# FEDDLib/FEDDLib

Hardware: AMD Instinct MI355X
Metric: DoF/s assemble+solve, 3D P1-Laplace cube (higher is better)
Workload: dtype f64

## Files before the change

feddlib_amd/csrc/gmres.hip:

```cpp
#include "fedd_internal.hpp"
#include <rccl/rccl.h>
#include <algorithm>
#include <cmath>
#include <cstdlib>

namespace fedd {
namespace {

constexpr int MD_ROWS = 2048;
constexpr int MD_CG = 8;
constexpr int MD2_CG = 8;
constexpr int AX_ROWS = 512;

__device__ __forceinline__ double2 ld2c(const double* __restrict__ p, int64_t r, int64_t n) {
    if (r + 1 < n) return *reinterpret_cast<const double2*>(p + r);
    double2 v;
    v.x = r < n ? p[r] : 0.0;
    v.y = 0.0;
    return v;
}

__device__ __forceinline__ double2 ld2(const double* __restrict__ p, int64_t r, int64_t n) {
    if (r + 1 < n) {
        typedef double v2d __attribute__((ext_vector_type(2)));
// ... 718 lines not shown
    double* V = f.V;
    double* u = f.w0;
    double* wt = f.w1;
    double* r = f.r;
    const dim3 gn = f.gn, blk = f.blk;
    hipStream_t st = f.st;

    FEDD_TRY(f.start(wt, -1));
    if (!(f.beta0 > 0)) {
        f.report(its_out, relres_out);
        return 0;
    }
    LaggedCheck lag(f, 2);
    FEDD_TRY(lag.create());
    const int nblkd = (int)((n + 2047) / 2048);
    const int md2_gy = c->md2_gy > 0 ? c->md2_gy : (int)std::max<int64_t>(1, (2048 + nblkd - 1) / nblkd);
    bool converged = false;
    while (!converged && f.its < max_it) {
        hipLaunchKernelGGL(k_cycle_init, dim3(1), dim3(1), 0, st, S, o, m, (const double*)(S + o.nrm + 3));
        hipLaunchKernelGGL(k_scale_to, gn, blk, 0, st, (const double*)r, (const double*)(S + o.misc + 1), V, n);
        FEDD_TRY(f.apply(V, u));
        {
            ScopedTimer t(c, FEDD_T_ORTHO);
            hipLaunchKernelGGL(k_multidot, dim3(nblk, 1), blk, 0, st, (const double*)V, ldv, n, 1, (const double*)u,
                               c->d_part.p, nblk, (const int32_t*)nullptr);
            hipLaunchKernelGGL(k_reduce_cols, dim3(1), blk, 0, st, (const double*)c->d_part.p, S + o2.hp, nblk,
                               (const int32_t*)nullptr);
            FEDD_TRY(allreduce_sum(c, S + o2.hp, 1));
            hipLaunchKernelGGL(k_multiaxpy, dim3(nblk2), blk, 0, st, (const double*)V, ldv, n, 1, (const double*)(S + o2.hp),
                               u, c->d_part.p, (const int32_t*)nullptr);
            t.stop();
        }
        lag.begin_cycle();
        int stop = 0;
        for (int j = 0; j < m && lag.issued < max_it && !stop; ++j) {
            const int k = j + 1;
            FEDD_TRY(f.apply(u, wt, true));
            {
                ScopedTimer t(c, FEDD_T_ORTHO);
                const int ncg = (k + 1 + MD2_CG - 1) / MD2_CG;
                ScopedTimer td(c, FEDD_T_GS_DOT);
                td.bytes(8.0 * (double)n * (k + 2));
                hipLaunchKernelGGL(k_multidot2<4>, dim3(nblkd, std::min(md2_gy, ncg)), blk, 0, st, (const double*)V, ldv, n,
                                   k, (const double*)u, (const double*)wt, c->d_part.p, nblkd);
                td.stop();
                hipLaunchKernelGGL(k_reduce_cols, dim3(2 * k + 2), blk, 0, st, (const double*)c->d_part.p, S + o2.st, nblkd,
                                   (const int32_t*)nullptr);
                FEDD_TRY(allreduce_sum(c, S + o2.st, 2 * k + 2));
                hipLaunchKernelGGL(k_dcgs2_small, dim3(1), blk, (size_t)(6 * m + 8) * sizeof(double), st, S, o, o2, k, m,
                                   c->h_pinned_dev ? c->h_pinned_dev + 4 * (j & 1) : (double*)nullptr);
                if (k < m) {
                    ScopedTimer tu(c, FEDD_T_GS_UPDATE);
                    tu.bytes(8.0 * (double)n * (k + 4));
                    hipLaunchKernelGGL(k_axpy2, dim3(nblk2), blk, 0, st, V, ldv, n, k, (const double*)(S + o2.cf), m, u,
                                       (const double*)wt);
                    tu.stop();
                }
                t.stop();
            }
            FEDD_TRY(lag.record(j, !c->h_pinned_dev, &stop));
        }
        FEDD_TRY(lag.drain(&stop));
        converged = stop == 1;
        const bool broke = stop == 2;
        FEDD_TRY(f.add_correction(lag.cols, call.x));
        if (!converged && (f.its < max_it || broke)) {
            FEDD_TRY(f.true_residual(call.x, r, false, -1, f.project));
            if (broke) {
                double ta = 0.0;
                FEDD_TRY(f.read_norm(&ta));
                f.relres = ta / f.beta0;
                if (f.relres <= call.rtol) converged = true;
            }
        }
    }
    return f.finish(its_out, relres_out);
}


constexpr int ss_cg(int S) { return S >= 16 ? 2 : 4; }

template <int OFF>
__device__ __forceinline__ double xchg_add(double lo, double hi, int lane) {
    if constexpr (OFF == 32 || OFF == 16) {
        const unsigned l0 = __double2loint(lo), l1 = __double2hiint(lo), h0 = __double2loint(hi), h1 = __double2hiint(hi);
        if constexpr (OFF == 32) {
            const auto r0 = __builtin_amdgcn_permlane32_swap(l0, h0, false, false);
            const auto r1 = __builtin_amdgcn_permlane32_swap(l1, h1, false, false);
            return __hiloint2double(r1[0], r0[0]) + __hiloint2double(r1[1], r0[1]);
        } else {
            const auto r0 = __builtin_amdgcn_permlane16_swap(l0, h0, false, false);
            const auto r1 = __builtin_amdgcn_permlane16_swap(l1, h1, false, false);
            return __hiloint2double(r1[0], r0[0]) + __hiloint2double(r1[1], r0[1]);
        }
    } else {
        const bool up = (lane & OFF) != 0;
        const double keep = up ? hi : lo;
        const double send = up ? lo : hi;
        return keep + __shfl_xor(send, OFF, 64);
    }
}

template <int NV, int OFF, int W>
__device__ __forceinline__ void wave_reduce_step(double (&a)[NV], int lane) {
    if constexpr (W > 1) {
#pragma unroll
        for (int i = 0; i < W / 2; ++i) a[i] = xchg_add<OFF>(a[i], a[i + W / 2], lane);
    } else {
        a[0] += __shfl_xor(a[0], OFF, 64);
    }
    if constexpr (OFF > 1) wave_reduce_step<NV, OFF / 2, (W > 1 ? W / 2 : 1)>(a, lane);
}
template <int NV>
__device__ __forceinline__ double wave_reduce_transpose(double (&a)[NV], int lane) {
    wave_reduce_step<NV, 32, NV>(a, lane);
    return a[0];
}

struct RowPair {
    int64_t rc;
    bool v0, v1;
};
__device__ __forceinline__ RowPair row_pair(int64_t r, int64_t n) {
    RowPair q;
    q.v0 = r < n;
    q.v1 = r + 1 < n;
    q.rc = q.v0 ? r : 0;
    return q;
}
template <bool NT>
__device__ __forceinline__ double2 ldraw(const double* __restrict__ p, const RowPair& q) {
    typedef double v2d __attribute__((ext_vector_type(2)));
    const v2d t = NT ? __builtin_nontemporal_load(reinterpret_cast<const v2d*>(p + q.rc)) : *reinterpret_cast<const v2d*>(p + q.rc);
    return double2{t.x, t.y};
}
template <bool NT>
__device__ __forceinline__ double2 ldp(const double* __restrict__ p, const RowPair& q) {
    typedef double v2d __attribute__((ext_vector_type(2)));
    const v2d t = NT ? __builtin_nontemporal_load(reinterpret_cast<const v2d*>(p + q.rc)) : *reinterpret_cast<const v2d*>(p + q.rc);
    double2 v;
    v.x = q.v0 ? t.x : 0.0;
    v.y = q.v1 ? t.y : 0.0;
    return v;
}

constexpr int SS_LDS_GROUPS = 32;

template <int S, int NCH, int SS_CG>
__global__ __launch_bounds__(256) void k_blockdot(const double* __restrict__ V, int64_t ldv, int64_t n, int k, int sa_req,
                                                  const int32_t* __restrict__ d_sa, double* __restrict__ partial, int nblk) {
    constexpr int NV = SS_CG * S;
    static_assert(NV == 16 || NV == 32 || NV == 64, "block size");
    __shared__ double sh[SS_LDS_GROUPS][4][NV];
    const int sa = d_sa ? min(*d_sa, sa_req) : sa_req;
    if (sa <= 0) return;
    const int tid = threadIdx.x, lane = tid & 63, wave = tid >> 6;
    const int half = tid / 256, th = tid % 256;
    RowPair rp[NCH];
#pragma unroll
    for (int ch = 0; ch < NCH; ++ch)
        rp[ch] = row_pair((int64_t)blockIdx.x * (512 * NCH) + 512 * ch + 2 * th, n);
    double2 w[S][NCH];
#pragma unroll
    for (int j = 0; j < S; ++j)
#pragma unroll
        for (int ch = 0; ch < NCH; ++ch) {
            const int jj = half * S + j;
            const double2 t = ldp<false>(V + (int64_t)(k + (jj < sa ? jj : 0)) * ldv, rp[ch]);
            w[j][ch].x = jj < sa ? t.x : 0.0;
            w[j][ch].y = jj < sa ? t.y : 0.0;
        }
    const int ncol = k + sa;
    const int ncg = (ncol + SS_CG - 1) / SS_CG;
    int parked = 0, first_cg = blockIdx.y;
    constexpr int GRP = 64 / NV;
    auto flush = [&](int count) {
        __syncthreads();
        for (int e = tid; e < count * NV; e += 256) {
            const int g = e / NV, idx = e % NV;
            const int col = (first_cg + g * (int)gridDim.y) * SS_CG + idx / S;
            if (col < ncol) partial[((int64_t)col * S + (idx % S)) * nblk + blockIdx.x] = ((sh[g][0][idx] + sh[g][1][idx]) + sh[g][2][idx]) + sh[g][3][idx];
        }
        __syncthreads();
    };
    double2 v[SS_CG][NCH];
    auto load_group = [&](int cg) {
#pragma unroll
        for (int cc = 0; cc < SS_CG; ++cc) {
            const int col = cg * SS_CG + cc;
            const double* __restrict__ a = V + (int64_t)(col < ncol ? col : 0) * ldv;
#pragma unroll
            for (int ch = 0; ch < NCH; ++ch) {
                v[cc][ch] = col < k ? ldraw<true>(a, rp[ch]) : ldraw<false>(a, rp[ch]);
            }
        }
    };
    if ((int)blockIdx.y < ncg) load_group(blockIdx.y);
    for (int cg = blockIdx.y; cg < ncg; cg += gridDim.y) {
        double acc[NV];
#pragma unroll
        for (int cc = 0; cc < SS_CG; ++cc)
#pragma unroll
            for (int j = 0; j < S; ++j) {
                double s = 0.0;
#pragma unroll
                for (int ch = 0; ch < NCH; ++ch) s += v[cc][ch].x * w[j][ch].x + v[cc][ch].y * w[j][ch].y;
                acc[cc * S + j] = s;
            }
        if (cg + (int)gridDim.y < ncg) load_group(cg + gridDim.y);
        const double tot = wave_reduce_transpose<NV>(acc, lane);
        if ((lane & (GRP - 1)) == 0) sh[parked][wave][lane / GRP] = tot;
        if (++parked == SS_LDS_GROUPS) {
            flush(parked);
            parked = 0;
            first_cg = cg + gridDim.y;
        }
    }
    if (parked) flush(parked);
}

template <int S, bool COMB = false>
__global__ __launch_bounds__(256) void k_blockaxpy(double* __restrict__ V, int64_t ldv, int64_t n, int k, int sa_req,
                                                   const int32_t* __restrict__ d_sa, const double* __restrict__ cf,
                                                   const double* __restrict__ rinv, const double* __restrict__ yv = nullptr,
                                                   double* __restrict__ comb = nullptr) {
    const int sa = min(*d_sa, sa_req);
    if (sa <= 0) return;
    const int tid = threadIdx.x;
    const int64_t r = (int64_t)blockIdx.x * AX_ROWS + 2 * tid;
    const RowPair rp = row_pair(r, n);
    double2 cb = double2{0.0, 0.0};
    double2 acc[S];
#pragma unroll
    for (int j = 0; j < S; ++j) acc[j] = double2{0.0, 0.0};
    int c = 0;
    for (; c + 8 <= k; c += 8) {
        double2 q[8];
#pragma unroll
        for (int u = 0; u < 8; ++u) q[u] = ldp<true>(V + (int64_t)(c + u) * ldv, rp);
#pragma unroll
        for (int u = 0; u < 8; ++u) {
#pragma unroll
            for (int j = 0; j < S; ++j) {
                const double cc = cf[(c + u) * S + j];
                acc[j].x += cc * q[u].x;
                acc[j].y += cc * q[u].y;
            }
            if constexpr (COMB) {
                const double yc = yv[c + u];
                cb.x += yc * q[u].x;
                cb.y += yc * q[u].y;
            }
        }
    }
    for (; c < k; ++c) {
        const double2 q = ldp<true>(V + (int64_t)c * ldv, rp);
#pragma unroll
        for (int j = 0; j < S; ++j) {
            const double cc = cf[c * S + j];
            acc[j].x += cc * q.x;
            acc[j].y += cc * q.y;
        }
        if constexpr (COMB) {
            const double yc = yv[c];
            cb.x += yc * q.x;
            cb.y += yc * q.y;
        }
    }
    double2 t[S];
#pragma unroll
    for (int j = 0; j < S; ++j) {
        const double2 wv = ldp<false>(V + (int64_t)(k + (j < sa ? j : 0)) * ldv, rp);
        t[j].x = j < sa ? wv.x - acc[j].x : 0.0;
        t[j].y = j < sa ? wv.y - acc[j].y : 0.0;
    }
#pragma unroll
    for (int j = 0; j < S; ++j) {
        if (j < sa) {
            double2 o = double2{0.0, 0.0};
#pragma unroll
            for (int i = 0; i <= j; ++i) {
                const double ri = rinv[i * S + j];
                o.x += ri * t[i].x;
                o.y += ri * t[i].y;
            }
            double* wj = V + (int64_t)(k + j) * ldv;
            if (rp.v1) *reinterpret_cast<double2*>(wj + r) = o;
            else if (rp.v0) wj[r] = o.x;
            if constexpr (COMB) {
                if (j < sa - 1) {
                    const double yc = yv[k + j];
                    cb.x += yc * o.x;
                    cb.y += yc * o.y;
                }
            }
        }
    }
    if constexpr (COMB) {
        if (rp.v1) *reinterpret_cast<double2*>(comb + r) = cb;
        else if (rp.v0) comb[r] = cb.x;
    }
}

template <int S>
__global__ __launch_bounds__(256) void k_blockfuse(double* __restrict__ V, int64_t ldv, int64_t n, int k, int sa_req,
                                                   const int32_t* __restrict__ d_sa, const double* __restrict__ cf,
                                                   const double* __restrict__ rinv, double* __restrict__ partial, int nblk) {
    constexpr int SS_CG = 2, NV = SS_CG * S;
    static_assert(NV == 32, "block size");
    __shared__ double sh[SS_LDS_GROUPS][4][NV];
    const int sa = min(*d_sa, sa_req);
    if (sa <= 0) return;
    const int tid = threadIdx.x, lane = tid & 63, wave = tid >> 6;
    const int64_t r = (int64_t)blockIdx.x * AX_ROWS + 2 * tid;
    const RowPair rp = row_pair(r, n);
    double2 w[S];
    {
        double2 acc[S];
#pragma unroll
        for (int j = 0; j < S; ++j) acc[j] = double2{0.0, 0.0};
        int c = 0;
        for (; c + 8 <= k; c += 8) {
            double2 q[8];
#pragma unroll
            for (int u = 0; u < 8; ++u) q[u] = ldp<false>(V + (int64_t)(c + u) * ldv, rp);
#pragma unroll
            for (int u = 0; u < 8; ++u)
#pragma unroll
                for (int j = 0; j < S; ++j) {
                    const double cc = cf[(c + u) * S + j];
                    acc[j].x += cc * q[u].x;
                    acc[j].y += cc * q[u].y;
                }
        }
        for (; c < k; ++c) {
            const double2 q = ldp<false>(V + (int64_t)c * ldv, rp);
#pragma unroll
            for (int j = 0; j < S; ++j) {
                const double cc = cf[c * S + j];
                acc[j].x += cc * q.x;
                acc[j].y += cc * q.y;
            }
        }
#pragma unroll
        for (int j = 0; j < S; ++j) {
            const double2 wv = ldp<false>(V + (int64_t)(k + (j < sa ? j : 0)) * ldv, rp);
            acc[j].x = j < sa ? wv.x - acc[j].x : 0.0;
            acc[j].y = j < sa ? wv.y - acc[j].y : 0.0;
        }
#pragma unroll
        for (int j = 0; j < S; ++j) {
            double2 o = double2{0.0, 0.0};
            if (j < sa) {
#pragma unroll
                for (int i = 0; i <= j; ++i) {
                    const double ri = rinv[i * S + j];
                    o.x += ri * acc[i].x;
                    o.y += ri * acc[i].y;
                }
                double* wj = V + (int64_t)(k + j) * ldv;
                if (rp.v1) *reinterpret_cast<double2*>(wj + r) = o;
                else if (rp.v0) wj[r] = o.x;
            }
            w[j] = o;
        }
    }
    const int ncol = k + sa;
    const int ncg = (ncol + SS_CG - 1) / SS_CG;
    int parked = 0, first_cg = 0;
    constexpr int GRP = 64 / NV;
    auto flush = [&](int count) {
        __syncthreads();
        for (int e = tid; e < count * NV; e += 256) {
            const int g = e / NV, idx = e % NV;
            const int col = (first_cg + g) * SS_CG + idx / S;
            if (col < ncol) partial[((int64_t)col * S + (idx % S)) * nblk + blockIdx.x] = ((sh[g][0][idx] + sh[g][1][idx]) + sh[g][2][idx]) + sh[g][3][idx];
        }
        __syncthreads();
    };
    double2 v[SS_CG];
    auto load_group = [&](int cg) {
#pragma unroll
        for (int cc = 0; cc < SS_CG; ++cc) {
            const int col = cg * SS_CG + cc;
            const double* __restrict__ a = V + (int64_t)(col < ncol ? col : 0) * ldv;
            v[cc] = col < k ? ldraw<true>(a, rp) : ldp<false>(a, rp);
        }
    };
    load_group(0);
    for (int cg = 0; cg < ncg; ++cg) {
        double acc[NV];
#pragma unroll
        for (int cc = 0; cc < SS_CG; ++cc)
#pragma unroll
            for (int j = 0; j < S; ++j) acc[cc * S + j] = v[cc].x * w[j].x + v[cc].y * w[j].y;
        if (cg + 1 < ncg) load_group(cg + 1);
        const double tot = wave_reduce_transpose<NV>(acc, lane);
        if ((lane & (GRP - 1)) == 0) sh[parked][wave][lane / GRP] = tot;
        if (++parked == SS_LDS_GROUPS) {
            flush(parked);
            parked = 0;
            first_cg = cg + 1;
        }
    }
    if (parked) flush(parked);
}

struct Off3 {
    int Hraw, P, C1, R1, R1i, Cc, cf1, ri1, cf2, ri2, th, res;
};

template <int S>
__device__ int chol_cut(double (&A)[S][S], const double* gdiag, int sa, double tol, double (&W)[S][S], double (&R)[S][S],
                        double (&Ri)[S][S], double* dd, int* s_ok, int tid) {
    const int i = tid / S, j = tid % S;
    if (tid < S) dd[tid] = (tid < sa && A[tid][tid] > 0.0) ? sqrt(A[tid][tid]) : 0.0;
    if (tid == 0) *s_ok = sa;
    __syncthreads();
    if (tid < S * S) {
        W[i][j] = (i <= j && dd[i] > 0.0 && dd[j] > 0.0) ? A[i][j] / (dd[i] * dd[j]) : 0.0;
        R[i][j] = 0.0;
        Ri[i][j] = 0.0;
    }
    __syncthreads();
    for (int c = 0; c < sa; ++c) {
        if (tid == 0) {
            const double piv = W[c][c];
            if (!(dd[c] > 0.0) || !(piv > 0.0) || !(piv * A[c][c] > tol * gdiag[c])) *s_ok = c;
        }
        __syncthreads();
        if (*s_ok <= c) break;
        const double rp = 1.0 / sqrt(W[c][c]);
        __syncthreads();
        if (tid < S && tid >= c) R[c][tid] = W[c][tid] * rp;
        __syncthreads();
        if (tid < S * S && i > c && i <= j) W[i][j] -= R[c][i] * R[c][j];
        __syncthreads();
    }
    const int ok = *s_ok;
    if (tid < S * S) R[i][j] = (i <= j && j < ok) ? R[i][j] * dd[j] : 0.0;
    __syncthreads();
    if (tid < ok) {
        const int cj = tid;
        Ri[cj][cj] = 1.0 / R[cj][cj];
        for (int r = cj - 1; r >= 0; --r) {
            double acc = 0.0;
            for (int p = r + 1; p <= cj; ++p) acc += R[r][p] * Ri[p][cj];
            Ri[r][cj] = -acc / R[r][r];
        }
    }
    __syncthreads();
    return ok;
}

template <int S>
__device__ void gram_minus(const double* __restrict__ P, int k, double (&G)[S][S], double (&A)[S][S], int tid) {
    if (tid < S * S) {
        const int i = tid / S, j = tid % S;
        double s0 = 0.0, s1 = 0.0, s2 = 0.0, s3 = 0.0;
        int c = 0;
        for (; c + 4 <= k; c += 4) {
            s0 += P[(c + 0) * S + i] * P[(c + 0) * S + j];
            s1 += P[(c + 1) * S + i] * P[(c + 1) * S + j];
            s2 += P[(c + 2) * S + i] * P[(c + 2) * S + j];
            s3 += P[(c + 3) * S + i] * P[(c + 3) * S + j];
        }
        for (; c < k; ++c) s0 += P[c * S + i] * P[c * S + j];
        const double g = P[(k + i) * S + j];
        G[i][j] = g;
        A[i][j] = g - ((s0 + s1) + (s2 + s3));
    }
}

template <int S>
__global__ __launch_bounds__(256) void k_ss_pass1(double* __restrict__ Sx, Off3 o3, int k, int sa_req, double tol,
                                                  int32_t* __restrict__ d_sa) {
    __shared__ double G[S][S], A[S][S], W[S][S], R[S][S], Ri[S][S];
    __shared__ double gd[S], dd[S];
    __shared__ int s_ok;
    const int tid = threadIdx.x;
    const double* P = Sx + o3.P;
    gram_minus<S>(P, k, G, A, tid);
    __syncthreads();
    if (tid < S) gd[tid] = G[tid][tid];
    __syncthreads();
    const int ok1 = chol_cut<S>(A, gd, sa_req, tol, W, R, Ri, dd, &s_ok, tid);
    if (tid == 0) d_sa[0] = ok1;
    __syncthreads();
    for (int i = tid; i < k * S; i += 256) {
        const double v = P[i];
        Sx[o3.C1 + i] = v;
        Sx[o3.cf1 + i] = v;
    }
    if (tid < S * S) {
        Sx[o3.R1 + tid] = R[tid / S][tid % S];
        Sx[o3.R1i + tid] = Ri[tid / S][tid % S];
        Sx[o3.ri1 + tid] = Ri[tid / S][tid % S];
    }
}

template <int S>
__global__ __launch_bounds__(256) void k_ss_pass2(double* __restrict__ Sx, Off o, Off3 o3, int k, int sa_req, int m, double tol,
                                                  int32_t* __restrict__ d_sa, double* __restrict__ host_out) {
    extern __shared__ double dyn[];
    __shared__ double G[S][S], A[S][S], W[S][S], R2[S][S], R2i[S][S], R1[S][S], R1i[S][S], Rc[S][S], Rci[S][S];
    __shared__ double gd[S], th[S], dd[S];
    __shared__ int s_sa;
    double* hc = dyn;
    double* lcs = hc + (size_t)S * (m + 2);
    double* lsn = lcs + m;
    const int tid = threadIdx.x, ldh = m + 1;
    const double* P = Sx + o3.P;
    double* Hraw = Sx + o3.Hraw;
    const int sa1 = min(d_sa[0], sa_req);
    if (tid < S * S) {
        R1[tid / S][tid % S] = Sx[o3.R1 + tid];
        R1i[tid / S][tid % S] = Sx[o3.R1i + tid];
    }
    if (tid < S) th[tid] = Sx[o3.th + tid];
    for (int i = tid; i < k - 1; i += 256) {
        lcs[i] = Sx[o.cs + i];
        lsn[i] = Sx[o.sn + i];
    }
    int sa = 0;
    if (sa1 > 0) {
        gram_minus<S>(P, k, G, A, tid);
        __syncthreads();
        if (tid < S) gd[tid] = G[tid][tid];
        __syncthreads();
        sa = chol_cut<S>(A, gd, sa1, tol, W, R2, R2i, dd, &s_sa, tid);
    }
    __syncthreads();
    const bool brk = sa == 0;
    if (!brk) {
        if (tid < S * S) {
            const int i = tid / S, j = tid % S;
            double s = 0.0, t = 0.0;
            for (int p = 0; p < S; ++p) {
                s += R2[i][p] * R1[p][j];
                t += R1i[i][p] * R2i[p][j];
            }
            Rc[i][j] = (i < sa && j < sa) ? s : 0.0;
            Rci[i][j] = (i < sa && j < sa) ? t : 0.0;
        }
        for (int idx = tid; idx < k * S; idx += 256) {
            const int cc = idx / S, j = idx % S;
            double s = Sx[o3.C1 + idx];
            for (int i = 0; i <= j; ++i) s += P[cc * S + i] * R1[i][j];
            Sx[o3.Cc + idx] = s;
            Sx[o3.cf2 + idx] = P[idx];
        }
        if (tid < S * S) Sx[o3.ri2 + tid] = R2i[tid / S][tid % S];
    } else {
        for (int idx = tid; idx < k * S; idx += 256) Sx[o3.Cc + idx] = Sx[o3.C1 + idx];
        if (tid < S * S) Rc[tid / S][tid % S] = 0.0;
    }
    __syncthreads();
    for (int cidx = tid; cidx <= k; cidx += 256) {
        const double v = cidx < k ? Sx[o3.Cc + cidx * S] + (cidx == k - 1 ? th[0] : 0.0) : Rc[0][0];
        Hraw[(int64_t)(k - 1) * ldh + cidx] = v;
    }
    __syncthreads();
    const int nc = brk ? 0 : sa - 1;
    if (nc > 0) {
        for (int r = tid; r < k + sa; r += 256) {
            double x[S];
#pragma unroll
            for (int cidx = 0; cidx < S; ++cidx) x[cidx] = 0.0;
            for (int q0 = 0; q0 < k; q0 += 8) {
                double h[8];
#pragma unroll
                for (int u = 0; u < 8; ++u) {
                    const int q = q0 + u;
                    h[u] = (q < k && r <= k && q + 1 >= r) ? Hraw[(int64_t)q * ldh + r] : 0.0;
                }
#pragma unroll
                for (int u = 0; u < 8; ++u) {
                    const int q = q0 + u;
                    if (q < k) {
#pragma unroll
                        for (int cidx = 0; cidx < S - 1; ++cidx) x[cidx] -= h[u] * Sx[o3.Cc + q * S + cidx];
                    }
                }
            }
#pragma unroll
            for (int cidx = 0; cidx < S - 1; ++cidx) {
                if (cidx < nc) {
                    if (r < k) x[cidx] += Sx[o3.Cc + r * S + cidx + 1] + th[cidx + 1] * Sx[o3.Cc + r * S + cidx];
                    else x[cidx] += Rc[r - k][cidx + 1] + th[cidx + 1] * Rc[r - k][cidx];
                }
            }
#pragma unroll
            for (int cidx = 0; cidx < S - 1; ++cidx) {
                if (cidx < nc && r <= k + cidx + 1) {
                    double hv = 0.0;
#pragma unroll
                    for (int cp = 0; cp < S - 1; ++cp)
                        if (cp <= cidx) hv += x[cp] * Rci[cp][cidx];
                    Hraw[(int64_t)(k + cidx) * ldh + r] = hv;
                }
            }
        }
    }
    __syncthreads();
    const int ncolH = brk ? 1 : sa;
    for (int i = 0; i < ncolH; ++i) {
        const int jj = k - 1 + i;
        double* hci = hc + (size_t)i * (m + 2);
        for (int q = tid; q <= jj + 1; q += 256) hci[q] = Hraw[(int64_t)jj * ldh + q];
    }
    __syncthreads();
    if (tid < ncolH) {
        double* hci = hc + (size_t)tid * (m + 2);
        for (int q = 0; q < k - 1; ++q) {
            const double a = lcs[q] * hci[q] + lsn[q] * hci[q + 1];
            hci[q + 1] = -lsn[q] * hci[q] + lcs[q] * hci[q + 1];
            hci[q] = a;
        }
    }
    __syncthreads();
    if (tid == 0) {
        for (int i = 0; i < ncolH; ++i) {
            const int jj = k - 1 + i;
            double* hci = hc + (size_t)i * (m + 2);
            for (int q = k - 1; q < jj; ++q) {
                const double a = lcs[q] * hci[q] + lsn[q] * hci[q + 1];
                hci[q + 1] = -lsn[q] * hci[q] + lcs[q] * hci[q + 1];
                hci[q] = a;
            }
            const double d = hypot(hci[jj], hci[jj + 1]);
            const double cj = d > 0 ? hci[jj] / d : 1.0, sj = d > 0 ? hci[jj + 1] / d : 0.0;
            lcs[jj] = cj;
            lsn[jj] = sj;
            Sx[o.cs + jj] = cj;
            Sx[o.sn + jj] = sj;
            hci[jj] = d;
            hci[jj + 1] = 0.0;
            const double gj = Sx[o.g + jj];
            Sx[o.g + jj + 1] = -sj * gj;
            Sx[o.g + jj] = cj * gj;
            Sx[o3.res + i] = fabs(sj * gj);
        }
    }
    __syncthreads();
    for (int i = 0; i < ncolH; ++i) {
        const int jj = k - 1 + i;
        const double* hci = hc + (size_t)i * (m + 2);
        double* H = Sx + o.H + (int64_t)jj * ldh;
        for (int q = tid; q <= jj + 1; q += 256) H[q] = hci[q];
    }
    __syncthreads();
    if (tid == 0) {
        d_sa[0] = sa;
        Sx[o.misc + 4] = (double)sa;
        Sx[o.misc + 5] = brk ? 1.0 : 0.0;
        if (host_out) {
            host_out[0] = (double)sa;
            host_out[1] = brk ? 1.0 : 0.0;
            for (int i = 0; i < S; ++i) host_out[2 + i] = i < ncolH ? Sx[o3.res + i] : 0.0;
            __threadfence_system();
        }
    }
}

__global__ void k_ss_cycle_init(double* __restrict__ S, Off o, Off3 o3, int m, int s, const double* __restrict__ rr) {
    const double beta = sqrt(rr[0]);
    for (int i = threadIdx.x; i <= m; i += blockDim.x) S[o.g + i] = 0.0;
    __syncthreads();
    if (threadIdx.x == 0) {
        S[o.g] = beta;
        S[o.misc + 1] = beta > 0 ? 1.0 / beta : 0.0;
        S[o.misc + 3] = beta;
    }
}

static void hessenberg_real_parts(std::vector<double> H, int n, int ld, double* out) {
    std::vector<double> cs((size_t)n), sn((size_t)n);
    auto at = [&](int i, int j) -> double& { return H[(size_t)j * ld + i]; };
    for (int sweep = 0; sweep < 500; ++sweep) {
        for (int i = 0; i + 1 < n; ++i) {
            const double a = at(i, i), b = at(i + 1, i), d = std::hypot(a, b);
            cs[i] = d > 0 ? a / d : 1.0;
            sn[i] = d > 0 ? b / d : 0.0;
            for (int j = i; j < n; ++j) {
                const double u = at(i, j), v = at(i + 1, j);
                at(i, j) = cs[i] * u + sn[i] * v;
                at(i + 1, j) = -sn[i] * u + cs[i] * v;
            }
        }
        for (int i = 0; i + 1 < n; ++i)
            for (int r = 0; r <= std::min(i + 1, n - 1); ++r) {
                const double u = at(r, i), v = at(r, i + 1);
                at(r, i) = cs[i] * u + sn[i] * v;
                at(r, i + 1) = -sn[i] * u + cs[i] * v;
            }
    }
    for (int i = 0; i < n;) {
        const double sub = i + 1 < n ? std::fabs(at(i + 1, i)) : 0.0;
        if (i + 1 < n && sub > 1e-10 * (std::fabs(at(i, i)) + std::fabs(at(i + 1, i + 1)))) {
            const double a = at(i, i), b = at(i, i + 1), c2 = at(i + 1, i), d = at(i + 1, i + 1);
            const double tr = 0.5 * (a + d), disc = 0.25 * (a - d) * (a - d) + b * c2;
            const double rt = disc > 0.0 ? std::sqrt(disc) : 0.0;
            out[i] = tr + rt;
            out[i + 1] = tr - rt;
            i += 2;
        } else {
            out[i] = at(i, i);
            ++i;
        }
    }
}

static void leja_order(double* v, int n) {
    std::vector<double> in(v, v + n), out;
    std::vector<char> used((size_t)n, 0);
    for (int t = 0; t < n; ++t) {
        int best = -1;
        double bestv = -1e300;
        for (int i = 0; i < n; ++i) {
            if (used[(size_t)i]) continue;
            double score = 0.0;
            if (out.empty()) score = std::fabs(in[(size_t)i]);
            else for (double o : out) score += std::log(std::max(std::fabs(in[(size_t)i] - o), 1e-300));
            if (score > bestv) {
                bestv = score;
                best = i;
            }
        }
        used[(size_t)best] = 1;
        out.push_back(in[(size_t)best]);
    }
    std::copy(out.begin(), out.end(), v);
}

template <int S>
static int gmres_solve_sstep(fedd_ctx* c, const GmresCall& call, int s, int* its_out, double* relres_out) {
    Frame f;
    FEDD_TRY(f.setup(c, call, true));
    const int nr = f.nr;
    FEDD_CHECK(nr == 1 || (nr == MULTI_NR && call.use_prec && multi_rhs_ok(c)), "gmres: stacked solve with %d right-hand sides", nr);
    const int64_t n = f.n, ldv = f.ldv;
    const int m = f.m, nblk = f.nblk, nblk2 = f.nblk2, max_it = call.max_it;
    const double rtol = call.rtol;
    constexpr int dot_cg = ss_cg(S);
    const int nblkd = (int)((n + 1023) / 1024);
    const Off o = f.o;
    Off3 o3;
    o3.Hraw = f.p; f.p += (m + 1) * m;
    o3.P = f.p; f.p += (m + 1 + S) * S;
    o3.C1 = f.p; f.p += m * S;
    o3.Cc = f.p; f.p += m * S;
    o3.cf1 = f.p; f.p += m * S;
    o3.cf2 = f.p; f.p += m * S;
    o3.R1 = f.p; f.p += S * S;
    o3.R1i = f.p; f.p += S * S;
    o3.ri1 = f.p; f.p += S * S;
    o3.ri2 = f.p; f.p += S * S;
    o3.th = f.p; f.p += S;
    o3.res = f.p; f.p += S;
    FEDD_TRY(f.alloc(std::max((size_t)(m + 1 + S) * S * (c->gmres_fuse != 0 ? std::max(nblkd, nblk2) : nblkd), (size_t)std::max(nblk, nblk2)), true));
    FEDD_TRY(c->d_flags.ensure(16));
    double* Sx = f.S;
    double* V = f.V;
    double* xt = f.w0;
    double* axt = f.w1;
    double* r = f.r;
    double* d_x = call.x;
    int32_t* d_sa = c->d_flags.p + 12;
    const dim3 gn = f.gn, blk = f.blk;
    hipStream_t st = f.st;
    const double chol_tol = c->gmres_chol_tol;
    const size_t pass2_lds = (size_t)(S * (m + 2) + 2 * m) * sizeof(double);
    FEDD_CHECK(pass2_lds <= 128 * 1024, "gmres (s-step): restart length %d with blocks of %d vectors exceeds the LDS of the block kernel", m, S);
    if (pass2_lds > 40 * 1024)
        FEDD_HIP(hipFuncSetAttribute((const void*)k_ss_pass2<S>, hipFuncAttributeMaxDynamicSharedMemorySize, (int)pass2_lds));

    const double* mk = f.mk;
    FEDD_HIP(hipMemsetAsync(Sx + o3.th, 0, (size_t)S * sizeof(double), st));
    FEDD_TRY(f.start(axt, 0));
    if (!(f.beta0 > 0)) {
        f.report(its_out, relres_out);
        return 0;
    }
    const double beta0 = f.beta0;
    const bool project = f.project;
    int& its = f.its;
    double& relres = f.relres;
    hipEvent_t ev = nullptr;
    FEDD_HIP(hipEventCreateWithFlags(&ev, hipEventDisableTiming));
    struct EvGuard {
        hipEvent_t e;
        ~EvGuard() { (void)hipEventDestroy(e); }
    } ev_guard{ev};
    const int gy_dot = c->gmres_dot_gy > 0 ? c->gmres_dot_gy
                                           : (int)std::max<int64_t>(1, std::min<int64_t>(4, (1024 + nblkd / 2) / std::max(nblkd, 1)));
    double* hout = c->h_pinned + 16;
    double* hout_dev = c->h_pinned_dev ? c->h_pinned_dev + 16 : nullptr;

    int precomb_cols = -1;
    auto trial = [&](int cols, double* true_abs) -> int {
        if (cols > 0) {
            FEDD_TRY(f.add_correction(cols, xt, cols == precomb_cols));
            precomb_cols = -1;
        } else {
            FEDD_HIP(hipMemcpyAsync(xt, d_x, (size_t)n * sizeof(double), hipMemcpyDeviceToDevice, st));
        }
        FEDD_TRY(f.true_residual(xt, axt, true, 0, false));
        return f.read_norm(true_abs);
    };
    auto commit = [&]() -> int {
        FEDD_HIP(hipMemcpyAsync(d_x, xt, (size_t)n * sizeof(double), hipMemcpyDeviceToDevice, st));
        return 0;
    };

    const int s_tol = !c->gmres_tol_blocks || rtol >= 1e-9 ? 16 : (rtol >= 1e-11 ? 5 : 3);
    const int s_goal = std::max(1, std::min(std::min(s, S), s_tol));
    const bool newton = c->gmres_newton && s_goal > 8 && !mk && nr == 1;
    bool have_shifts = false;
    std::vector<double> theta((size_t)S, 0.0);
    int s_cur = std::min(s_goal, 8);
    const bool dbg = getenv("FEDD_GMRES_DEBUG") != nullptr;
    if (dbg) fprintf(stderr, "[gmres s-step] basis at %p (%zu MB), ldv %lld\n", (void*)V, c->d_V.cap * sizeof(double) >> 20, (long long)ldv);
    double tol_abs = rtol * beta0;
    double last_true = beta0;
    int floor_restarts = 0;
    int nfail = 0;
    double best_fail = 1e300;
    int stalls = 0;
    bool done = false;
    c->gmres_blocks = 0;
    c->gmres_cut_blocks = 0;
    c->gmres_fused_blocks = 0;
    bool first_cycle = true;
    while (!done && its < max_it) {
        if (project && !first_cycle) {
            double ta = 0.0;
            FEDD_TRY(coarse_apply_add(c, r, d_x));
            FEDD_TRY(trial(0, &ta));
            last_true = ta;
            relres = ta / beta0;
        }
        first_cycle = false;
        hipLaunchKernelGGL(k_ss_cycle_init, dim3(1), dim3(256), 0, st, Sx, o, o3, m, S, (const double*)(Sx + o.nrm + 3));
        hipLaunchKernelGGL(k_scale_to, gn, blk, 0, st, (const double*)r, (const double*)(Sx + o.misc + 1), V, n);
        int k = 1;
        bool restart_now = false;
        int spec_done = 0, spec_k = -1;
        while (!done && !restart_now) {
            const int room = std::min(m - (k - 1), max_it - its - (k - 1));
            if (room <= 0) break;
            const int sa = std::min(s_cur, room);
            const int i0 = spec_k == k ? std::min(spec_done, sa) : 0;
            spec_done = 0;
            spec_k = -1;
            for (int i = i0; i < sa; ++i)
                FEDD_TRY(f.apply(V + (int64_t)(k - 1 + i) * ldv, V + (int64_t)(k + i) * ldv, false, have_shifts ? theta[(size_t)i] : 0.0));
            {
                ScopedTimer t(c, FEDD_T_ORTHO);
                const int ncg = (k + sa + dot_cg - 1) / dot_cg;
                const dim3 gd(nblkd, std::min(gy_dot, ncg));
                auto launch_dot = [&](const int32_t* dsa) {
                    hipLaunchKernelGGL((k_blockdot<S, 2, dot_cg>), gd, blk, 0, st, (const double*)V, ldv, n, k, sa, dsa, c->d_part.p, nblkd);
                };
                const double dot_bytes = 8.0 * (double)n * (k + 2 * sa), upd_bytes = 8.0 * (double)n * (k + 2 * sa);
                {
                    ScopedTimer td(c, FEDD_T_GS_DOT);
                    td.bytes(dot_bytes);
                    launch_dot((const int32_t*)nullptr);
                }
                hipLaunchKernelGGL(k_reduce_cols, dim3((k + sa) * S), blk, 0, st, (const double*)c->d_part.p, Sx + o3.P, nblkd,
                                   (const int32_t*)nullptr);
                FEDD_TRY(allreduce_sum(c, Sx + o3.P, (k + sa) * S));
                hipLaunchKernelGGL(k_ss_pass1<S>, dim3(1), blk, 0, st, Sx, o3, k, sa, chol_tol, d_sa);
                bool fused = false;
                if constexpr (S == 16) fused = c->gmres_fuse > 0 || (c->gmres_fuse < 0 && n >= 4000000);
                if (fused) {
                    ++c->gmres_fused_blocks;
                    if constexpr (S == 16) {
                        ScopedTimer tu(c, FEDD_T_GS_FUSED);
                        tu.bytes(upd_bytes);
                        hipLaunchKernelGGL(k_blockfuse<S>, dim3(nblk2), blk, 0, st, V, ldv, n, k, sa, (const int32_t*)d_sa,
                                           (const double*)(Sx + o3.cf1), (const double*)(Sx + o3.ri1), c->d_part.p, nblk2);
                    }
                } else {
                    {
                        ScopedTimer tu(c, FEDD_T_GS_UPDATE);
                        tu.bytes(upd_bytes);
                        hipLaunchKernelGGL(k_blockaxpy<S>, dim3(nblk2), blk, 0, st, V, ldv, n, k, sa, (const int32_t*)d_sa,
                                           (const double*)(Sx + o3.cf1), (const double*)(Sx + o3.ri1));
                    }
                    {
                        ScopedTimer td(c, FEDD_T_GS_DOT);
                        td.bytes(dot_bytes);
                        launch_dot((const int32_t*)d_sa);
                    }
                }
                hipLaunchKernelGGL(k_reduce_cols, dim3((k + sa) * S), blk, 0, st, (const double*)c->d_part.p, Sx + o3.P, fused ? nblk2 : nblkd,
                                   (const int32_t*)nullptr);
                FEDD_TRY(allreduce_sum(c, Sx + o3.P, (k + sa) * S));
                hipLaunchKernelGGL(k_ss_pass2<S>, dim3(1), blk, pass2_lds, st, Sx, o, o3, k, sa, m,
                                   chol_tol, d_sa, hout_dev);
                if (!hout_dev) {
                    FEDD_HIP(hipMemcpyAsync(hout, Sx + o.misc + 4, 2 * sizeof(double), hipMemcpyDeviceToHost, st));
                    FEDD_HIP(hipMemcpyAsync(hout + 2, Sx + o3.res, S * sizeof(double), hipMemcpyDeviceToHost, st));
                }
                FEDD_HIP(hipEventRecord(ev, st));
                bool comb = false;
                if constexpr (S == 16) comb = c->gmres_fuse != 0 && nr == 1 && k - 1 + sa == m && sa >= 2;
                precomb_cols = -1;
                if (comb) {
                    if constexpr (S == 16) {
                        hipLaunchKernelGGL(k_backsolve, dim3(1), dim3(256), (size_t)(k + sa) * sizeof(double), st, Sx, o, k - 1 + sa, m);
                        ScopedTimer tu(c, FEDD_T_GS_UPDATE);
                        tu.bytes(upd_bytes + 8.0 * (double)n);
                        hipLaunchKernelGGL((k_blockaxpy<S, true>), dim3(nblk2), blk, 0, st, V, ldv, n, k, sa, (const int32_t*)d_sa,
                                           (const double*)(Sx + o3.cf2), (const double*)(Sx + o3.ri2), (const double*)(Sx + o.y), r);
                        precomb_cols = k - 1 + sa;
                    }
                } else {
                    ScopedTimer tu(c, FEDD_T_GS_UPDATE);
                    tu.bytes(upd_bytes);
                    hipLaunchKernelGGL(k_blockaxpy<S>, dim3(nblk2), blk, 0, st, V, ldv, n, k, sa, (const int32_t*)d_sa,
                                       (const double*)(Sx + o3.cf2), (const double*)(Sx + o3.ri2));
                }
                t.stop();
            }
            if (c->gmres_spec > 0 && !(newton && !have_shifts)) {
                const int k_next = k + sa;
                const int room_next = std::min(m - (k_next - 1), max_it - its - (k_next - 1));
                const int ns = std::min(std::min(c->gmres_spec, s_cur), room_next);
                for (int i = 0; i < ns; ++i)
                    FEDD_TRY(f.apply(V + (int64_t)(k_next - 1 + i) * ldv, V + (int64_t)(k_next + i) * ldv, false, have_shifts ? theta[(size_t)i] : 0.0));
                if (ns > 0) {
                    spec_done = ns;
                    spec_k = k_next;
                }
            }
            FEDD_HIP(hipEventSynchronize(ev));
            const int sa_eff = (int)hout[0];
            const bool brk = hout[1] != 0.0;
            const int ncolH = brk ? 1 : sa_eff;
            ++c->gmres_blocks;
            if (sa_eff < sa) ++c->gmres_cut_blocks;
            if (sa_eff < sa || brk) precomb_cols = -1;
            FEDD_CHECK(ncolH >= 1 && ncolH <= S, "gmres (s-step): block result %d", ncolH);
            for (int i = 0; i < ncolH && !done && !restart_now; ++i) {
                relres = hout[2 + i] / beta0;
                if (hout[2 + i] <= tol_abs) {
                    const int cols = k - 1 + i + 1;
                    double ta = 0.0;
                    FEDD_TRY(trial(cols, &ta));
                    if (dbg) fprintf(stderr, "[gmres s-step] k %d block col %d: claim with %d columns, recurrence %.3e true %.3e target %.3e (s %d)\n",
                                     k, i, cols, hout[2 + i] / beta0, ta / beta0, rtol, s_cur);
                    if (ta <= rtol * beta0) {
                        FEDD_TRY(commit());
                        its += cols;
                        relres = ta / beta0;
                        done = true;
                    } else if (nfail >= 1 && ta >= 0.5 * best_fail && ta <= 100.0 * rtol * beta0 && floor_restarts < 1) {
                        ++floor_restarts;
                        if (ta < last_true) {
                            FEDD_TRY(commit());
                            last_true = ta;
                        } else {
                            FEDD_TRY(trial(0, &ta));
                        }
                        its += cols;
                        relres = last_true / beta0;
                        nfail = 0;
                        best_fail = 1e300;
                        tol_abs = rtol * beta0;
                        restart_now = true;
                    } else if (nfail >= 1 && ta >= 0.5 * best_fail && ta <= 100.0 * rtol * beta0) {
                        FEDD_TRY(commit());
                        its += cols;
                        relres = ta / beta0;
                        c->gmres_floor = 1;
                        c->gmres_rec_relres = hout[2 + i] / beta0;
                        done = true;
                    } else if (ta > 4.0 * std::max(hout[2 + i], 1e-300) || !(ta < last_true)) {
                        ++nfail;
                        best_fail = std::min(best_fail, ta);
                        if (ta < last_true) {
                            FEDD_TRY(commit());
                            last_true = ta;
                            its += cols;
                        } else {
                            FEDD_TRY(trial(0, &ta));
                            its += cols;
                            ++stalls;
                        }
                        relres = last_true / beta0;
                        s_cur = std::max(1, s_cur / 2);
                        restart_now = true;
                    } else {
                        ++nfail;
                        best_fail = std::min(best_fail, ta);
                        tol_abs *= 0.9 * rtol * beta0 / ta;
                    }
                }
            }
            if (done || restart_now) break;
            if (brk) {
                double ta = 0.0;
                FEDD_TRY(trial(k, &ta));
                its += k;
                if (ta < last_true) {
                    FEDD_TRY(commit());
                    last_true = ta;
                } else {
                    FEDD_TRY(trial(0, &ta));
                    ++stalls;
                }
                relres = last_true / beta0;
                if (last_true <= rtol * beta0) done = true;
                restart_now = true;
                break;
            }
            k += sa_eff;
            if (sa_eff < sa) s_cur = std::max(1, sa_eff);
            else if (newton && !have_shifts && k - 1 >= s_goal) {
                std::vector<double> Hh((size_t)s_goal * s_goal);
                FEDD_HIP(hipMemcpy2DAsync(Hh.data(), (size_t)s_goal * sizeof(double), Sx + o3.Hraw, (size_t)(m + 1) * sizeof(double),
                                          (size_t)s_goal * sizeof(double), (size_t)s_goal, hipMemcpyDeviceToHost, st));
                FEDD_HIP(hipStreamSynchronize(st));
                hessenberg_real_parts(Hh, s_goal, s_goal, theta.data());
                leja_order(theta.data(), s_goal);
                bool finite = true;
                for (int i = 0; i < s_goal; ++i) finite = finite && std::isfinite(theta[(size_t)i]);
                if (finite) {
                    for (int i = 0; i < S; ++i) c->h_pinned[64 + i] = i < s_goal ? theta[(size_t)i] : 0.0;
                    FEDD_HIP(hipMemcpyAsync(Sx + o3.th, c->h_pinned + 64, (size_t)S * sizeof(double), hipMemcpyHostToDevice, st));
                    have_shifts = true;
                    s_cur = s_goal;
                    if (dbg) {
                        fprintf(stderr, "[gmres s-step] Newton shifts:");
                        for (int i = 0; i < s_goal; ++i) fprintf(stderr, " %.4f", theta[(size_t)i]);
                        fprintf(stderr, "\n");
                    }
                }
            }
        }
        if (done) break;
        if (!restart_now) {
            double ta = 0.0;
            FEDD_TRY(trial(k - 1, &ta));
            its += k - 1;
            if (ta < 0.999 * last_true) stalls = 0;
            else ++stalls;
            if (ta < last_true) {
                FEDD_TRY(commit());
                last_true = ta;
            } else {
                FEDD_TRY(trial(0, &ta));
            }
            relres = last_true / beta0;
            if (last_true <= rtol * beta0) done = true;
        }
        if (stalls >= 3) {
            c->gmres_floor = 2;
            break;
        }
    }
    return f.finish(its_out, relres_out);
}

static int gmres_solve_cgs2(fedd_ctx* c, const GmresCall& call, int* its_out, double* relres_out) {
    Frame f;
    FEDD_TRY(f.setup(c, call, false));
    const int64_t n = f.n, ldv = f.ldv;
    const int m = f.m, nblk = f.nblk, nblk2 = f.nblk2, max_it = call.max_it;
    const Off o = f.o;
    FEDD_TRY(f.alloc(std::max((size_t)(m + 2) * nblk, (size_t)nblk2), false));
    FEDD_TRY(c->d_flags.ensure(16));
    int32_t* gate = c->d_flags.p + 2;
    double* S = f.S;
    double* V = f.V;
    double* w = f.w0;
    double* r = f.r;
    const dim3 gn = f.gn, blk = f.blk;
    hipStream_t st = f.st;

    FEDD_TRY(f.start(r, -1));
    if (!(f.beta0 > 0)) {
        f.report(its_out, relres_out);
        return 0;
    }
    LaggedCheck lag(f, 1);
    FEDD_TRY(lag.create());
    int stop = 0;
    while (!stop && f.its < max_it) {
        hipLaunchKernelGGL(k_cycle_init, dim3(1), dim3(1), 0, st, S, o, m, (const double*)(S + o.nrm + 3));
        hipLaunchKernelGGL(k_scale_to, gn, blk, 0, st, (const double*)r, (const double*)(S + o.misc + 1), V, n);
        lag.begin_cycle();
        for (int j = 0; j < m && lag.issued < max_it && !stop; ++j) {
            FEDD_TRY(f.apply(V + (int64_t)j * ldv, w));
            {
                ScopedTimer t(c, FEDD_T_ORTHO);
                hipLaunchKernelGGL(k_multidot, dim3(nblk, (j + 2 + MD_CG - 1) / MD_CG), blk, 0, st, (const double*)V, ldv, n,
                                   j + 1, (const double*)w, c->d_part.p, nblk, (const int32_t*)nullptr);
                hipLaunchKernelGGL(k_reduce_cols, dim3(j + 2), blk, 0, st, (const double*)c->d_part.p, S + o.h1, nblk,
                                   (const int32_t*)nullptr);
                FEDD_TRY(allreduce_sum(c, S + o.h1, j + 2));
                hipLaunchKernelGGL(k_dgks_gate, dim3(1), dim3(1), 0, st, (const double*)(S + o.h1), j, gate, S + o.nrm + 1);
                hipLaunchKernelGGL(k_multiaxpy, dim3(nblk2), blk, 0, st, (const double*)V, ldv, n, j + 1,
                                   (const double*)(S + o.h1), w, c->d_part.p, (const int32_t*)nullptr);
                hipLaunchKernelGGL(k_multidot, dim3(nblk, (j + 2 + MD_CG - 1) / MD_CG), blk, 0, st, (const double*)V, ldv, n,
                                   j + 1, (const double*)w, c->d_part.p, nblk, (const int32_t*)gate);
                hipLaunchKernelGGL(k_reduce_cols, dim3(j + 1), blk, 0, st, (const double*)c->d_part.p, S + o.h2, nblk,
                                   (const int32_t*)gate);
                FEDD_TRY(allreduce_sum(c, S + o.h2, j + 1));
                hipLaunchKernelGGL(k_multiaxpy, dim3(nblk2), blk, 0, st, (const double*)V, ldv, n, j + 1,
                                   (const double*)(S + o.h2), w, c->d_part.p, (const int32_t*)gate);
                if (c->nranks > 1) {
                    hipLaunchKernelGGL(k_reduce_cols, dim3(1), blk, 0, st, (const double*)c->d_part.p, S + o.nrm + 2, nblk2,
                                       (const int32_t*)gate);
                    FEDD_TRY(allreduce_sum(c, S + o.nrm + 2, 1));
                }
                t.stop();
            }
            hipLaunchKernelGGL(k_givens, dim3(1), dim3(256), (size_t)(3 * m + 2) * sizeof(double), st, S, o, j, m,
                               (const int32_t*)gate, (const double*)(c->nranks > 1 ? nullptr : c->d_part.p), nblk2);
            hipLaunchKernelGGL(k_scale_to, gn, blk, 0, st, (const double*)w, (const double*)(S + o.misc + 1),
                               V + (int64_t)(j + 1) * ldv, n);
            FEDD_TRY(lag.record(j, true, &stop));
        }
        FEDD_TRY(lag.drain(&stop));
        FEDD_TRY(f.add_correction(lag.cols, call.x));
        if (!stop && f.its < max_it) FEDD_TRY(f.true_residual(call.x, r, false, -1, f.project));
    }
    return f.finish(its_out, relres_out);
}

int gmres_solve(fedd_ctx* c, const GmresCall& call, int* its_out, double* relres_out) {
    c->gmres_floor = 0;
    c->gmres_rec_relres = -1.0;
    FEDD_CHECK(call.nr <= 1 || c->gmres_kind == 2, "gmres: a stacked solve (%d right-hand sides) needs the s-step solver (gmres_kind 2)", call.nr);
    if (c->gmres_kind == 0) return gmres_solve_dcgs2(c, call, its_out, relres_out);
    if (c->gmres_kind == 1) return gmres_solve_cgs2(c, call, its_out, relres_out);
    int s = c->gmres_s;
    if (s == 0) {
        double ng = (double)c->n_rows;
        if (c->nranks > 1) {
            FEDD_TRY(c->d_small.ensure(std::max<size_t>(16, c->d_small.cap)));
            FEDD_HIP(hipMemcpyAsync(c->d_small.p, &ng, sizeof(double), hipMemcpyHostToDevice, c->stream));
            FEDD_HIP(hipStreamSynchronize(c->stream));
            FEDD_TRY(allreduce_sum(c, c->d_small.p, 1));
            FEDD_HIP(hipMemcpyAsync(&ng, c->d_small.p, sizeof(double), hipMemcpyDeviceToHost, c->stream));
            FEDD_HIP(hipStreamSynchronize(c->stream));
        }
        s = ng / c->nranks >= 1.2e6 ? 16 : 8;
    }
    c->gmres_s_used = s;
    if (s > 8 && (call.mask || std::min(call.restart, call.max_it) > 800)) s = 8;
    if (s <= 4) return gmres_solve_sstep<4>(c, call, s, its_out, relres_out);
    if (s <= 8) return gmres_solve_sstep<8>(c, call, s, its_out, relres_out);
    return gmres_solve_sstep<16>(c, call, s, its_out, relres_out);
}

}
```

Measured before the change: 111.6 million.

## Restructure fused block Gram-Schmidt kernel to stage row tiles in LDS

The fused update+dot kernel becomes a persistent grid sized to the CU count. Each block loops over 64-row sub-tiles, staging the V columns in dynamic LDS, and splits the 16 output vectors across waves (four per wave). The dot products are accumulated per thread across all tiles and written once per block, replacing the per-row-group wave reductions and partial flushes, and shrinking the partial buffer that the column reduction reads. The cost is more LDS traffic, extra barriers per tile, and fused-path eligibility that now depends on the restart length fitting in LDS.

```diff
diff --git a/feddlib_amd/csrc/gmres.hip b/feddlib_amd/csrc/gmres.hip
--- a/feddlib_amd/csrc/gmres.hip
+++ b/feddlib_amd/csrc/gmres.hip
@@ -1044,108 +1044,131 @@
     }
 }
 
+constexpr int FW_ROWS = 64;
+constexpr int FW_QS = FW_ROWS + 2;
+constexpr int FW_WS = 18;
+constexpr int FW_MAXCOL = 128;
+constexpr int FW_MAXWG = 4;
+inline size_t fw_lds_bytes(int k) { return ((size_t)(k + 16) * FW_QS + (size_t)FW_ROWS * FW_WS) * sizeof(double); }
+
 template <int S>
 __global__ __launch_bounds__(256) void k_blockfuse(double* __restrict__ V, int64_t ldv, int64_t n, int k, int sa_req,
                                                    const int32_t* __restrict__ d_sa, const double* __restrict__ cf,
                                                    const double* __restrict__ rinv, double* __restrict__ partial, int nblk) {
-    constexpr int SS_CG = 2, NV = SS_CG * S;
-    static_assert(NV == 32, "block size");
-    __shared__ double sh[SS_LDS_GROUPS][4][NV];
+    static_assert(S == 16, "block size");
+    extern __shared__ __align__(16) double fw_lds[];
     const int sa = min(*d_sa, sa_req);
     if (sa <= 0) return;
-    const int tid = threadIdx.x, lane = tid & 63, wave = tid >> 6;
-    const int64_t r = (int64_t)blockIdx.x * AX_ROWS + 2 * tid;
-    const RowPair rp = row_pair(r, n);
-    double2 w[S];
-    {
-        double2 acc[S];
-#pragma unroll
-        for (int j = 0; j < S; ++j) acc[j] = double2{0.0, 0.0};
-        int c = 0;
-        for (; c + 8 <= k; c += 8) {
+    double* Qs = fw_lds;
+    double* Wd = fw_lds + (size_t)(k + S) * FW_QS;
+    const int tid = threadIdx.x, lane = tid & 63;
+    const int wave = __builtin_amdgcn_readfirstlane(tid >> 6);
+    const int ncol = k + sa;
+    const int64_t nsub = (n + FW_ROWS - 1) / FW_ROWS;
+    const int sc = tid >> 5, sp = tid & 31;
+    const int j0 = 4 * wave;
+    const double* __restrict__ cfw = cf + j0;
+    const int jq = tid & 3, ca = tid >> 2, cb = ca + 64;
+    const double* xa_p = Qs + (ca < ncol ? ca : 0) * FW_QS;
+    const double* xb_p = Qs + (cb < ncol ? cb : 0) * FW_QS;
+    const double* wd_p = Wd + 4 * jq;
+    double da[4] = {0.0, 0.0, 0.0, 0.0}, db[4] = {0.0, 0.0, 0.0, 0.0};
+    for (int64_t sub = blockIdx.x; sub < nsub; sub += gridDim.x) {
+        const int64_t r0 = sub * FW_ROWS;
+        const RowPair rp = row_pair(r0 + 2 * sp, n);
+        for (int c0 = sc; c0 < k; c0 += 64) {
             double2 q[8];
 #pragma unroll
-            for (int u = 0; u < 8; ++u) q[u] = ldp<false>(V + (int64_t)(c + u) * ldv, rp);
-#pragma unroll
             for (int u = 0; u < 8; ++u)
-#pragma unroll
-                for (int j = 0; j < S; ++j) {
-                    const double cc = cf[(c + u) * S + j];
-                    acc[j].x += cc * q[u].x;
-                    acc[j].y += cc * q[u].y;
+                if (c0 + 8 * u < k) q[u] = ldraw<true>(V + (int64_t)(c0 + 8 * u) * ldv, rp);
+#pragma unroll
+            for (int u = 0; u < 8; ++u)
+                if (c0 + 8 * u < k) {
+                    double2 t;
+                    t.x = rp.v0 ? q[u].x : 0.0;
+                    t.y = rp.v1 ? q[u].y : 0.0;
+                    *reinterpret_cast<double2*>(Qs + (c0 + 8 * u) * FW_QS + 2 * sp) = t;
                 }
         }
-        for (; c < k; ++c) {
-            const double2 q = ldp<false>(V + (int64_t)c * ldv, rp);
-#pragma unroll
-            for (int j = 0; j < S; ++j) {
-                const double cc = cf[c * S + j];
-                acc[j].x += cc * q.x;
-                acc[j].y += cc * q.y;
-            }
-        }
-#pragma unroll
-        for (int j = 0; j < S; ++j) {
-            const double2 wv = ldp<false>(V + (int64_t)(k + (j < sa ? j : 0)) * ldv, rp);
-            acc[j].x = j < sa ? wv.x - acc[j].x : 0.0;
-            acc[j].y = j < sa ? wv.y - acc[j].y : 0.0;
-        }
-#pragma unroll
-        for (int j = 0; j < S; ++j) {
-            double2 o = double2{0.0, 0.0};
-            if (j < sa) {
-#pragma unroll
-                for (int i = 0; i <= j; ++i) {
-                    const double ri = rinv[i * S + j];
-                    o.x += ri * acc[i].x;
-                    o.y += ri * acc[i].y;
+        const int64_t r = r0 + lane;
+        const bool valid = r < n;
+        double wv[4];
+#pragma unroll
+        for (int jj = 0; jj < 4; ++jj)
+            wv[jj] = V[(int64_t)(k + (j0 + jj < sa ? j0 + jj : 0)) * ldv + (valid ? r : 0)];
+        __syncthreads();
+        {
+            double acc[4] = {0.0, 0.0, 0.0, 0.0};
+            const double* ql = Qs + lane;
+            int c = 0;
+            for (; c + 8 <= k; c += 8) {
+                double q[8], cc[8][4];
+#pragma unroll
+                for (int u = 0; u < 8; ++u) {
+                    q[u] = ql[(c + u) * FW_QS];
+#pragma unroll
+                    for (int jj = 0; jj < 4; ++jj) cc[u][jj] = cfw[(c + u) * S + jj];
                 }
-                double* wj = V + (int64_t)(k + j) * ldv;
-                if (rp.v1) *reinterpret_cast<double2*>(wj + r) = o;
-                else if (rp.v0) wj[r] = o.x;
-            }
-            w[j] = o;
-        }
-    }
-    const int ncol = k + sa;
-    const int ncg = (ncol + SS_CG - 1) / SS_CG;
-    int parked = 0, first_cg = 0;
-    constexpr int GRP = 64 / NV;
-    auto flush = [&](int count) {
+#pragma unroll
+                for (int u = 0; u < 8; ++u)
+#pragma unroll
+                    for (int jj = 0; jj < 4; ++jj) acc[jj] += cc[u][jj] * q[u];
+            }
+            for (; c < k; ++c) {
+                const double q = ql[c * FW_QS];
+#pragma unroll
+                for (int jj = 0; jj < 4; ++jj) acc[jj] += cfw[c * S + jj] * q;
+            }
+#pragma unroll
+            for (int jj = 0; jj < 4; ++jj) Qs[(k + j0 + jj) * FW_QS + lane] = (valid && j0 + jj < sa) ? wv[jj] - acc[jj] : 0.0;
+        }
         __syncthreads();
-        for (int e = tid; e < count * NV; e += 256) {
-            const int g = e / NV, idx = e % NV;
-            const int col = (first_cg + g) * SS_CG + idx / S;
-            if (col < ncol) partial[((int64_t)col * S + (idx % S)) * nblk + blockIdx.x] = ((sh[g][0][idx] + sh[g][1][idx]) + sh[g][2][idx]) + sh[g][3][idx];
-        }
+        double o[4] = {0.0, 0.0, 0.0, 0.0};
+#pragma unroll
+        for (int h = 0; h < S / 8; ++h)
+            if (8 * h <= j0 + 3) {
+                double t[8], rr[8][4];
+#pragma unroll
+                for (int u = 0; u < 8; ++u) {
+                    t[u] = Qs[(k + 8 * h + u) * FW_QS + lane];
+#pragma unroll
+                    for (int jj = 0; jj < 4; ++jj) rr[u][jj] = rinv[(8 * h + u) * S + j0 + jj];
+                }
+#pragma unroll
+                for (int u = 0; u < 8; ++u)
+#pragma unroll
+                    for (int jj = 0; jj < 4; ++jj) o[jj] += (8 * h + u <= j0 + jj ? rr[u][jj] : 0.0) * t[u];
+            }
         __syncthreads();
-    };
-    double2 v[SS_CG];
-    auto load_group = [&](int cg) {
-#pragma unroll
-        for (int cc = 0; cc < SS_CG; ++cc) {
-            const int col = cg * SS_CG + cc;
-            const double* __restrict__ a = V + (int64_t)(col < ncol ? col : 0) * ldv;
-            v[cc] = col < k ? ldraw<true>(a, rp) : ldp<false>(a, rp);
-        }
-    };
-    load_group(0);
-    for (int cg = 0; cg < ncg; ++cg) {
-        double acc[NV];
-#pragma unroll
-        for (int cc = 0; cc < SS_CG; ++cc)
-#pragma unroll
-            for (int j = 0; j < S; ++j) acc[cc * S + j] = v[cc].x * w[j].x + v[cc].y * w[j].y;
-        if (cg + 1 < ncg) load_group(cg + 1);
-        const double tot = wave_reduce_transpose<NV>(acc, lane);
-        if ((lane & (GRP - 1)) == 0) sh[parked][wave][lane / GRP] = tot;
-        if (++parked == SS_LDS_GROUPS) {
-            flush(parked);
-            parked = 0;
-            first_cg = cg + 1;
-        }
-    }
-    if (parked) flush(parked);
+#pragma unroll
+        for (int jj = 0; jj < 4; ++jj) {
+            const int j = j0 + jj;
+            const double ov = j < sa ? o[jj] : 0.0;
+            if (valid && j < sa) V[(int64_t)(k + j) * ldv + r] = ov;
+            Qs[(k + j) * FW_QS + lane] = ov;
+            Wd[lane * FW_WS + j] = ov;
+        }
+        __syncthreads();
+#pragma unroll 4
+        for (int p = 0; p < FW_ROWS / 2; ++p) {
+            const double2 xa = *reinterpret_cast<const double2*>(xa_p + 2 * p);
+            const double2 xb = *reinterpret_cast<const double2*>(xb_p + 2 * p);
+            const double2 w00 = *reinterpret_cast<const double2*>(wd_p + (2 * p) * FW_WS);
+            const double2 w01 = *reinterpret_cast<const double2*>(wd_p + (2 * p) * FW_WS + 2);
+            const double2 w10 = *reinterpret_cast<const double2*>(wd_p + (2 * p + 1) * FW_WS);
+            const double2 w11 = *reinterpret_cast<const double2*>(wd_p + (2 * p + 1) * FW_WS + 2);
+            da[0] += xa.x * w00.x; da[1] += xa.x * w00.y; da[2] += xa.x * w01.x; da[3] += xa.x * w01.y;
+            db[0] += xb.x * w00.x; db[1] += xb.x * w00.y; db[2] += xb.x * w01.x; db[3] += xb.x * w01.y;
+            da[0] += xa.y * w10.x; da[1] += xa.y * w10.y; da[2] += xa.y * w11.x; da[3] += xa.y * w11.y;
+            db[0] += xb.y * w10.x; db[1] += xb.y * w10.y; db[2] += xb.y * w11.x; db[3] += xb.y * w11.y;
+        }
+        __syncthreads();
+    }
+#pragma unroll
+    for (int jj = 0; jj < 4; ++jj) {
+        if (ca < ncol) partial[((int64_t)ca * S + 4 * jq + jj) * nblk + blockIdx.x] = da[jj];
+        if (cb < ncol) partial[((int64_t)cb * S + 4 * jq + jj) * nblk + blockIdx.x] = db[jj];
+    }
 }
 
 struct Off3 {
@@ -1500,7 +1523,19 @@
     o3.ri2 = f.p; f.p += S * S;
     o3.th = f.p; f.p += S;
     o3.res = f.p; f.p += S;
-    FEDD_TRY(f.alloc(std::max((size_t)(m + 1 + S) * S * (c->gmres_fuse != 0 ? std::max(nblkd, nblk2) : nblkd), (size_t)std::max(nblk, nblk2)), true));
+    bool fuse_ok = false;
+    int fw_cus = 0;
+    if constexpr (S == 16) {
+        if (c->gmres_fuse != 0 && m + 1 <= FW_MAXCOL) {
+            int dev = 0;
+            FEDD_HIP(hipGetDevice(&dev));
+            FEDD_HIP(hipDeviceGetAttribute(&fw_cus, hipDeviceAttributeMultiprocessorCount, dev));
+            FEDD_HIP(hipFuncSetAttribute((const void*)k_blockfuse<S>, hipFuncAttributeMaxDynamicSharedMemorySize, (int)fw_lds_bytes(m)));
+            fuse_ok = fw_cus > 0;
+        }
+    }
+    auto fw_grid = [&](int k) { return fw_cus * (int)std::max<size_t>(1, std::min<size_t>(FW_MAXWG, (size_t)160 * 1024 / fw_lds_bytes(k))); };
+    FEDD_TRY(f.alloc(std::max((size_t)(m + 1 + S) * S * (fuse_ok ? std::max(nblkd, FW_MAXWG * fw_cus) : nblkd), (size_t)std::max(nblk, nblk2)), true));
     FEDD_TRY(c->d_flags.ensure(16));
     double* Sx = f.S;
     double* V = f.V;
@@ -1615,14 +1650,15 @@
                 FEDD_TRY(allreduce_sum(c, Sx + o3.P, (k + sa) * S));
                 hipLaunchKernelGGL(k_ss_pass1<S>, dim3(1), blk, 0, st, Sx, o3, k, sa, chol_tol, d_sa);
                 bool fused = false;
-                if constexpr (S == 16) fused = c->gmres_fuse > 0 || (c->gmres_fuse < 0 && n >= 4000000);
+                if constexpr (S == 16) fused = fuse_ok && (c->gmres_fuse > 0 || (c->gmres_fuse < 0 && n >= 4000000));
+                const int nblkf = fused ? fw_grid(k) : 0;
                 if (fused) {
                     ++c->gmres_fused_blocks;
                     if constexpr (S == 16) {
                         ScopedTimer tu(c, FEDD_T_GS_FUSED);
                         tu.bytes(upd_bytes);
-                        hipLaunchKernelGGL(k_blockfuse<S>, dim3(nblk2), blk, 0, st, V, ldv, n, k, sa, (const int32_t*)d_sa,
-                                           (const double*)(Sx + o3.cf1), (const double*)(Sx + o3.ri1), c->d_part.p, nblk2);
+                        hipLaunchKernelGGL(k_blockfuse<S>, dim3(nblkf), blk, fw_lds_bytes(k), st, V, ldv, n, k, sa, (const int32_t*)d_sa,
+                                           (const double*)(Sx + o3.cf1), (const double*)(Sx + o3.ri1), c->d_part.p, nblkf);
                     }
                 } else {
                     {
@@ -1637,7 +1673,7 @@
                         launch_dot((const int32_t*)d_sa);
                     }
                 }
-                hipLaunchKernelGGL(k_reduce_cols, dim3((k + sa) * S), blk, 0, st, (const double*)c->d_part.p, Sx + o3.P, fused ? nblk2 : nblkd,
+                hipLaunchKernelGGL(k_reduce_cols, dim3((k + sa) * S), blk, 0, st, (const double*)c->d_part.p, Sx + o3.P, fused ? nblkf : nblkd,
                                    (const int32_t*)nullptr);
                 FEDD_TRY(allreduce_sum(c, Sx + o3.P, (k + sa) * S));
                 hipLaunchKernelGGL(k_ss_pass2<S>, dim3(1), blk, pass2_lds, st, Sx, o, o3, k, sa, m,
```

Measured after the change: 109.1 million. -2.2%, worse.
